# RIKEN-RCCS/GEMMul8

Hardware: AMD Instinct MI355X
Metric: emulated DGEMM TFLOPS (N=8192, moduli=14) (higher is better)
Workload: dtype int8

## Files before the change

### gemmul8_amd/csrc/oz2_driver.hip

```cpp
#include <hip/hip_runtime.h>
#include <stdint.h>
#include <stdio.h>
#include <stdlib.h>
#include <string.h>

#include <algorithm>

#include <atomic>
#include <mutex>

#include "../../include/gemmul8_c.h"
#include "oz2_gemm_common.hpp"
#include "oz2_kernels.h"
#include "oz2_knobs.hpp"

using namespace oz2;

namespace {

inline char* align256(void* p) {
    uintptr_t x = reinterpret_cast<uintptr_t>(p);
    x = (x + 255) & ~uintptr_t(255);
    return reinterpret_cast<char*>(x);
}
inline int norm_op(int op) {
    if (op >= 111 && op <= 113) return op - 111;
    return op;
}
inline size_t low_size(int) { return 1; }
inline size_t mid_size(int backend, bool cplx) { return (backend == kINT8 ? 1 : 2) * (cplx ? 2 : 1); }

static inline bool moduli_ok(int dtype, unsigned N) { return N >= 2 && N <= (is_f32(dtype) ? 13u : 20u); }

static inline bool f8_concat_ok(size_t k, size_t m, size_t n, size_t kp) { return k <= 32768 && 2 * (m + n) * kp <= ((size_t)384 << 20); }

#define OZ2_HIP(expr)                       \
    do {                                    \
        hipError_t e__ = (expr);            \
        if (e__ != hipSuccess) return (int)e__; \
    } while (0)

struct Timer {
    hipEvent_t ev[4];
    bool made = false, ok = false;
};
Timer* thread_timer() {
    constexpr int kMaxDev = 64;
    static thread_local Timer t[kMaxDev];
    int dev = 0;
    if (hipGetDevice(&dev) != hipSuccess || dev < 0 || dev >= kMaxDev) return nullptr;
    Timer& T = t[dev];
    if (!T.made) {
        T.made = T.ok = true;
        for (auto& e : T.ev)
            if (hipEventCreate(&e) != hipSuccess) T.ok = false;
    }
    return T.ok ? &T : nullptr;
}

}

static bool scalars_on_device(const void* alpha);

namespace oz2 {
static Knobs parse_knobs() {
    Knobs k;
    auto num = [](const char* name, int dflt) {
        const char* s = getenv(name);
        return s && *s ? atoi(s) : dflt;
    };
    if (const char* e = getenv("GEMMUL8_EPI_NT"); e && (e[0] == '0' || e[0] == '1') && !e[1]) k.epi_nt = e[0] - '0';
    if (const int t = num("GEMMUL8_BOUND_TILE", 0); t == 128 || t == 256) k.bound_tile = t;
    if (num("GEMMUL8_CPLX_BOUND_LAUNCHES", 1) == 2) k.cplx_bound_launches = 2;
    if (const int c = num("GEMMUL8_CPLX_CHUNK", 0); c >= 1) k.cplx_chunk = c;
    if (const char* e = getenv("GEMMUL8_CRT_KERNEL")) k.crt_kernel = e[0] == 'd' ? 1 : e[0] == 'r' ? 2 : 0;
    if (const int c = num("GEMMUL8_GEMM_CUS", 0); c >= 8) k.gemm_cus = c & ~7;
    if (const char* e = getenv("GEMMUL8_FP8_FUSED"); e && e[0] == '0') k.fp8_fused = 0;
    if (const char* e = getenv("GEMMUL8_FP8_PLANES")) k.fp8_planes = e[0] == 'e' ? 1 : 0;
    if (const char* e = getenv("GEMMUL8_SCALE_FOLD"); e && e[0] == '0') k.scale_fold = 0;
    if (const char* e = getenv("GEMMUL8_BOUNDS_ONE_READ"); e && (e[0] == '0' || e[0] == '1') && !e[1]) k.bounds_one_read = e[0] - '0';
    if (const char* e = getenv("GEMMUL8_CRT_PANELS"); e && atoi(e) > 1) {
        k.crt_panels = std::min(atoi(e), 256);
        k.crt_panels_ring = e[strlen(e) - 1] == 'r';
    }
    if (const char* e = getenv("GEMMUL8_MAP_COLBLOCK"); e && *e) k.map_colblock = atoi(e) > 0 ? atoi(e) : 0;
    return k;
}
static std::atomic<const Knobs*> g_knobs{nullptr};
static std::mutex g_knobs_mtx;
void reload_knobs() {
    std::lock_guard<std::mutex> lk(g_knobs_mtx);
    g_knobs.store(new Knobs(parse_knobs()), std::memory_order_release);
}
const Knobs& knobs() {
    const Knobs* k = g_knobs.load(std::memory_order_acquire);
    if (!k) {
        std::lock_guard<std::mutex> lk(g_knobs_mtx);
        k = g_knobs.load(std::memory_order_acquire);
        if (!k) g_knobs.store(k = new Knobs(parse_knobs()), std::memory_order_release);
    }
    return *k;
}
}

extern "C" {

void gemmul8_reload_knobs(void) { oz2::reload_knobs(); }

static std::atomic<int> g_nonfinite_mode{0};
int gemmul8_set_nonfinite_mode(int mode) {
    if (mode < 0 || mode > 1) return GEMMUL8_E_ARG;
    return g_nonfinite_mode.exchange(mode);
}

int gemmul8_set_fp8_bound_mode(int mode) {
    if (mode < 0 || mode > 2) return GEMMUL8_E_ARG;
    const int old = get_f8_bound_mode();
    set_f8_bound_mode(mode);
    return old;
}

int gemmul8_abi_version(void) { return GEMMUL8_ABI_VERSION; }
size_t gemmul8_layout_bytes(void) { return sizeof(gemmul8_layout); }

const char* gemmul8_version(void) { return "gemmul8-mi355x 0.5 (gfx950; v_mfma_i32_16x16x64_i8 / v_mfma_scale_f32_16x16x128_f8f6f4, fused epilogues)"; }

size_t gemmul8_work_size(int is_complex, int backend, size_t m, size_t n, size_t k, unsigned N, int enA, int enB, size_t* wA,
                         size_t* wB) {
    const size_t kp = padding256(k), mp = padding256(m);
    const size_t sizeA = kp * mp, sizeB = kp * n, sizeC = mp * n;
    const size_t nm = num_mat(backend, N);
    const size_t parts = is_complex ? 3 : 1;
    const size_t midsz = mid_size(backend, is_complex != 0);
    const size_t nhi = (backend == kINT8 ? 1 : 3) * parts;
    const size_t lwork = size_t(1) << 25;
    size_t tA = 255, tB = 255, tC = 255;
    tA += sizeA * (nm + (enA ? 1 : 0)) * parts + 2 * mp;
    tB += sizeB * (nm + (enB ? 1 : 0)) * parts + 2 * padding256(n);
    tC += midsz * sizeC * (N - 1) + std::max(lwork, midsz * sizeC);
    tC += 4 * sizeC * nhi;
    if (wA) *wA = tA;
    if (wB) *wB = tB;
    return tA + tB + tC;
}

int gemmul8_get_layout(int dtype, int backend, size_t m, size_t n, size_t k, unsigned N, void* work, void* workA, void* workB,
                       int enA, int enB, gemmul8_layout* L) {
    if (!L || !work) return GEMMUL8_E_ARG;
    if (!moduli_ok(dtype, N)) return GEMMUL8_E_NUM_MODULI;
    const bool cplx = is_complex(dtype);
    memset(L, 0, sizeof(*L));
    L->kp = padding256(k);
    L->mp = padding256(m);
    L->num_mat = num_mat(backend, N);
    L->parts = cplx ? 3 : 1;
    L->sizeA = L->kp * L->mp;
    L->sizeB = L->kp * n;
    L->sizeC = L->mp * n;
    const size_t offsetA = L->sizeA * L->num_mat, offsetB = L->sizeB * L->num_mat;
    const size_t size_vecA = L->mp, size_vecB = padding256(n);
    char* w = align256(work);
    char* wa = workA ? align256(workA) : nullptr;
    char* wb = workB ? align256(workB) : nullptr;
    char* A_lo = wa ? wa : w;
    char* sftA = A_lo + L->parts * offsetA + (enA ? L->parts * L->sizeA : 0);
    char* B_lo = wb ? wb : (wa ? w : sftA + 2 * size_vecA);
    char* sftB = B_lo + L->parts * offsetB + (enB ? L->parts * L->sizeB : 0);
    char* C_mid = wb ? (wa ? w : sftA + 2 * size_vecA) : sftB + 2 * size_vecB;
    const size_t midsz = mid_size(backend, cplx);
    char* work_native = C_mid + (N - 1) * L->sizeC * midsz;
    const size_t native_sz = std::max(size_t(1) << 25, midsz * L->sizeC);
    char* C_hi = work_native + native_sz;
    const size_t hi_bytes = 4 * L->sizeC * (backend == kINT8 ? 1 : 3) * L->parts;
    L->A_lo = A_lo;
    L->B_lo = B_lo;
    L->part_strideA = offsetA;
    L->part_strideB = offsetB;
    L->A_bound = enA ? A_lo + L->parts * offsetA : A_lo;
    L->B_bound = enB ? B_lo + L->parts * offsetB : B_lo;
    L->sftA = reinterpret_cast<int16_t*>(sftA);
    L->sftB = reinterpret_cast<int16_t*>(sftB);
    L->C_mid = C_mid;
    const size_t tail = (native_sz - midsz * L->sizeC) & ~size_t(255);
    L->scratch = C_hi - tail;
    L->scratch_bytes = tail + hi_bytes;
    L->lo_format = (backend == kFP8 && !enA && !enB && f6_planes_ok(n)) ? 1 : 0;
    return GEMMUL8_OK;
}

static inline size_t scale_fixed_bytes(size_t mp, size_t np) { return (4 * (mp + np) + 2 * (mp + np) + 255) / 256 * 256; }
static inline size_t scale_scratch_bytes(size_t mp, size_t np) { return scale_fixed_bytes(mp, np) + 8 * (mp + np); }
static int scale_scratch(const gemmul8_layout* L, size_t n, int** rowmax, int** colmax, void** amax, int16_t** s0A = nullptr, int16_t** s0B = nullptr) {
    const size_t np = padding256(n);
    if (L->scratch_bytes < scale_scratch_bytes(L->mp, np)) return GEMMUL8_E_ARG;
    *rowmax = (int*)L->scratch;
    *colmax = *rowmax + L->mp;
    int16_t* s0 = (int16_t*)(*colmax + np);
    if (s0A) *s0A = s0;
    if (s0B) *s0B = s0 + L->mp;
    *amax = (char*)L->scratch + scale_fixed_bytes(L->mp, np);
    return GEMMUL8_OK;
}

static int bound_gemm_i8(hipStream_t stream, bool cplx, const gemmul8_layout* L, size_t m, size_t ncols, const int8_t* Ab, const int8_t* Bb, int* rowmax, int* colmax) {
    if (!cplx) {
        const int8_t* As[1] = {Ab};
        const int8_t* Bs[1] = {Bb};
        OZ2_HIP(launch_gemm_i8_max(stream, 1, As, Bs, L->kp, m, ncols, rowmax, colmax));
    } else {
        const int8_t* As[3] = {Ab, Ab + L->sizeA, Ab + 2 * L->sizeA};
        const int8_t* Bs[3] = {Bb + L->sizeB, Bb, Bb + 2 * L->sizeB};
        const bool two_launches = knobs().cplx_bound_launches == 2;
        if (two_launches) {
            OZ2_HIP(launch_gemm_i8_max(stream, 2, As, Bs, L->kp, m, ncols, rowmax, colmax));
            OZ2_HIP(launch_gemm_i8_max(stream, 3, As, Bs, L->kp, m, ncols, rowmax, colmax));
        } else {
            OZ2_HIP(launch_gemm_i8_max(stream, 3, As, Bs, L->kp, m, ncols, rowmax, colmax, 2));
        }
    }
    return GEMMUL8_OK;
}

struct SymSide {
    bool onB;
    int form;
    bool herm;
    bool conj = false;
};
constexpr size_t kOneReadMinRows = 8192;
static int scale_bounds_nf(void* stream_, int dtype, int backend, int op_A, int op_B, size_t m, size_t n, size_t k, const void* A, size_t lda,
                           const void* B, size_t ldb, unsigned N, size_t col_begin, size_t col_end, const gemmul8_layout* L, int skipA, int skipB,
                           bool nf, const SymSide* sym = nullptr) {
    hipStream_t stream = (hipStream_t)stream_;
    if (!L || !A || !B) return GEMMUL8_E_ARG;
    if (!moduli_ok(dtype, N)) return GEMMUL8_E_NUM_MODULI;
    if (backend == kFP8 && k > 65536) return GEMMUL8_E_ARG;
    op_A = norm_op(op_A);
// ... 911 lines not shown
```

### gemmul8_amd/csrc/oz2_gemm_i8.hip

```cpp
#include <hip/hip_runtime.h>
#include <stdint.h>

#include <atomic>
#include <cstdlib>
#include <type_traits>

#include "oz2_crt_common.hpp"
#include "oz2_gemm_common.hpp"
#include "oz2_gemm_i8_epi.hpp"
#include "oz2_kernels.h"

namespace oz2 {

#ifndef OZ2_PB
#define OZ2_PB 4
#endif
#ifndef OZ2_KBAR_MAX_KP
#define OZ2_KBAR_MAX_KP 5120
#endif
#ifndef OZ2_SLEEP_A
#define OZ2_SLEEP_A 4
#endif
#ifndef OZ2_SLEEP_B
#define OZ2_SLEEP_B 4
#endif
constexpr int RING_LDS_BYTES = 5 * TILE_BYTES;

struct NoCrt {
    int unused;
};
#ifdef OZ2_LAB_FUSED_CRT
#include OZ2_LAB_FUSED_CRT
#endif
template <bool ZERO> struct MfmaReinitHook {
    v4i (*acc)[4];
    int acc0;
    __device__ __forceinline__ void operator()(int sb, int phase) const {
        if (phase != 0) return;
        const int tj = sb >> 1, tg = sb & 1;
        const v4i z = {0, 0, 0, 0};
        const v4i c = ZERO ? v4i{0, 0, 0, 0} : v4i{acc0, acc0, acc0, acc0};
        __builtin_amdgcn_sched_barrier(0);
#pragma unroll
        for (int ti = 0; ti < 4; ++ti)
            acc[tg * 4 + ti][tj] = __builtin_amdgcn_mfma_i32_16x16x64_i8(z, acc[tg * 4 + ti][tj], c, 0, 0, 0);
    }
};
#define OZ2_I8_KR 0
#define OZ2_I8_KERNEL_HEAD                                       \
    template <int EPI, bool KBAR, int FUSE, bool SMALLK = false> \
    __global__ void __launch_bounds__(WS_THREADS) gemm_i8_kernel(const GemmArgs args, const std::conditional_t<FUSE != 0, CrtArgs, NoCrt> crt)
#include "oz2_gemm_i8_kernel.inc"
#undef OZ2_I8_KR
#undef OZ2_I8_KERNEL_HEAD
#define OZ2_I8_KR 1
#define OZ2_I8_KERNEL_HEAD                           \
    template <int EPI, bool KBAR, int FUSE, bool SMALLK> \
    __global__ void __launch_bounds__(WS_THREADS) gemm_i8_kr_kernel(const GemmArgs args, const NoCrt crt, const int krange)
#include "oz2_gemm_i8_kernel.inc"
#undef OZ2_I8_KR
#undef OZ2_I8_KERNEL_HEAD

static void fill_common(GemmArgs& a, size_t kp, size_t m, size_t n) {
    a.kp = (int)kp;
    a.m = (int)m;
    a.n = (int)n;
    a.tiles_m = (int)((m + BM - 1) / BM);
    a.tiles_n = (int)((n + BN - 1) / BN);
    for (int t = 0; t < 20; ++t) {
        const int p = GEMMUL8_MODULI_INT8[t];
        a.moduli[t] = p;
        a.pinv32[t] = (int)(4294967296ull / (unsigned long long)p);
        a.dotw[t] = 1u | ((256u % p) << 8) | ((65536u % p) << 16) | ((16777216u % p) << 24);
        a.dotc[t] = (unsigned)((p - (int)(2147483648u % (unsigned)p)) % p);
    }
}

static int num_cus() {
    static int n = 0;
    if (!n) {
        int dev = 0;
        hipDeviceProp_t prop;
        if (hipGetDevice(&dev) != hipSuccess || hipGetDeviceProperties(&prop, dev) != hipSuccess || prop.multiProcessorCount <= 0) return 256;
        n = prop.multiProcessorCount;
    }
    return n;
}

template <int EPI, bool KBAR, int FUSE = 0, bool SMALLK = false, bool KR = false>
static hipError_t launch_sched(hipStream_t stream, GemmArgs& a, const std::conditional_t<FUSE != 0, CrtArgs, NoCrt>& crt = {}, [[maybe_unused]] int krange = 0) {
    static std::atomic<bool> attr_set_dev[64];
    int dev_ = 0;
    if (hipGetDevice(&dev_) != hipSuccess || dev_ < 0 || dev_ >= 64) dev_ = 0;
    if (!attr_set_dev[dev_].load(std::memory_order_acquire)) {
        const void* fn;
        if constexpr (KR) fn = (const void*)gemm_i8_kr_kernel<EPI, KBAR, FUSE, SMALLK>;
        else fn = (const void*)gemm_i8_kernel<EPI, KBAR, FUSE, SMALLK>;
        hipError_t e = hipFuncSetAttribute(fn, hipFuncAttributeMaxDynamicSharedMemorySize, RING_LDS_BYTES);
        if (e != hipSuccess) return e;
        attr_set_dev[dev_].store(true, std::memory_order_release);
    }
    int grid = num_cus() & ~7;
    if (const int want = knobs().gemm_cus; want > 0 && want < grid) grid = want;
    if (grid <= 0) grid = 8;
    if (a.total_tiles < grid) grid = a.total_tiles;
    if constexpr (KR) hipLaunchKernelGGL((gemm_i8_kr_kernel<EPI, KBAR, FUSE, SMALLK>), dim3(grid), dim3(WS_THREADS), RING_LDS_BYTES, stream, a, crt, krange);
    else hipLaunchKernelGGL((gemm_i8_kernel<EPI, KBAR, FUSE, SMALLK>), dim3(grid), dim3(WS_THREADS), RING_LDS_BYTES, stream, a, crt);
    return hipGetLastError();
}

template <int EPI> static hipError_t launch(hipStream_t stream, GemmArgs& a, int planes, int tri = 0, int krange = 0) {
    a.ppi = planes;
    a.m_ppi = map_magic((unsigned)planes);
    a.bstride = g_batch.ws;
    planes *= (int)g_batch.batch;
    if (tri != 0 && (EPI == EPI_MAX || a.tiles_m != a.tiles_n)) return hipErrorInvalidValue;
    if (krange != 0 && (EPI == EPI_MAX || tri != 0 || a.nseg != 1 || g_batch.batch != 1 || krange < kKrALower || krange > kKrBLow)) return hipErrorInvalidValue;
    if (krange != 0 && (krange <= kKrAUpper ? a.tiles_m : a.tiles_n) != a.kp / 256) return hipErrorInvalidValue;
    a.total_tiles = tri ? planes * (a.tiles_m * (a.tiles_m + 1) / 2) : planes * a.tiles_m * a.tiles_n;
    if (a.total_tiles <= 0) return hipSuccess;
    a.colblock = tri ? 0 : map_colblock((size_t)a.tiles_n, (size_t)a.kp * (size_t)a.nseg);
    a.map = tri ? make_tile_map_tri(a.tiles_m, tri) : make_tile_map(a.tiles_m, a.tiles_n, a.colblock);
    a.acc0 = (size_t)a.kp * (size_t)a.nseg <= 512 ? 0 : (int)0x80000000u;
    if constexpr (EPI != EPI_MAX) {
        if (krange != 0) {
            if (a.acc0 == 0) return launch_sched<EPI, true, 0, true, true>(stream, a, {}, krange);
            if (a.kp <= OZ2_KBAR_MAX_KP) return launch_sched<EPI, true, 0, false, true>(stream, a, {}, krange);
            return launch_sched<EPI, false, 0, false, true>(stream, a, {}, krange);
        }
        if (a.acc0 == 0) return launch_sched<EPI, true, 0, true>(stream, a);
        if (a.kp * a.nseg <= OZ2_KBAR_MAX_KP) return launch_sched<EPI, true>(stream, a);
    }
    return launch_sched<EPI, false>(stream, a);
}

static int nt_residue_planes(const GemmArgs& a, int planes, bool stream_out, bool automatic = true) {
    if (const int force = knobs().epi_nt; force >= 0) return force == 1 && stream_out ? planes : 0;
    if (!stream_out || !automatic) return 0;
    const size_t all = (size_t)planes * g_batch.batch;
    const size_t operands = all * (a.strideA + a.strideB), residues = all * a.strideO;
    return residues >= ((size_t)256 << 20) && operands <= ((size_t)240 << 20) ? planes : 0;
}

hipError_t launch_gemm_i8_mod(hipStream_t stream, const int8_t* A, const int8_t* B, size_t strideA, size_t strideB, size_t kp, size_t m,
                              size_t n, int t_begin, int t_end, int8_t* out, size_t ldo, size_t strideO, bool stream_out, int tri, int krange) {
    GemmArgs a{};
    a.A[0] = A;
    a.B[0] = B;
    a.nseg = 1;
    a.strideA = strideA;
    a.strideB = strideB;
    a.t_begin = t_begin;
    a.out = out;
    a.ldo = ldo;
    a.strideO = strideO;
    fill_common(a, kp, m, n);
    a.nt_planes = nt_residue_planes(a, t_end - t_begin, stream_out);
    return launch<EPI_MOD>(stream, a, t_end - t_begin, tri, krange);
}

hipError_t launch_gemm_i8_cplx(hipStream_t stream, const int8_t* A, const int8_t* B, size_t strideA, size_t strideB, size_t kp, size_t m,
                               size_t n, int t_begin, int t_end, const int8_t* rx, const int8_t* ry, size_t strideR, int8_t* out,
                               size_t ldo, size_t strideO, int tri, int krange) {
    GemmArgs a{};
    a.A[0] = A;
    a.B[0] = B;
    a.nseg = 1;
    a.strideA = strideA;
    a.strideB = strideB;
    a.t_begin = t_begin;
    a.out = out;
    a.ldo = ldo;
    a.strideO = strideO;
    a.rx = rx;
    a.ry = ry;
    a.strideR = strideR;
    fill_common(a, kp, m, n);
    a.nt_planes = nt_residue_planes(a, t_end - t_begin, true, false);
    return launch<EPI_CPLX>(stream, a, t_end - t_begin, tri, krange);
}

#ifndef OZ2_MAX_SMALL_TILES
#define OZ2_MAX_SMALL_TILES 128
#endif
hipError_t launch_gemm_i8_max(hipStream_t stream, int nseg, const int8_t* const* A, const int8_t* const* B, size_t kp, size_t m, size_t n,
                              int* rowmax, int* colmax, int mid_seg) {
    {
        const int force = knobs().bound_tile;
        const size_t tiles = ((m + BM - 1) / BM) * ((n + BN - 1) / BN) * g_batch.batch;
        const bool small = force == 128 ? true : force == 256 ? false : tiles <= (size_t)OZ2_MAX_SMALL_TILES;
        if (small) return launch_gemm_i8_max_small(stream, nseg, A, B, kp, m, n, rowmax, colmax, mid_seg);
    }
    GemmArgs a{};
    for (int s = 0; s < nseg; ++s) a.A[s] = A[s], a.B[s] = B[s];
    a.nseg = nseg;
    a.rowmax = rowmax;
    a.colmax = colmax;
    a.kt_mid = mid_seg > 0 && mid_seg < nseg ? mid_seg * (int)(kp / BK) : 0;
    fill_common(a, kp, m, n);
    return launch<EPI_MAX>(stream, a, 1);
}

}
```

### gemmul8_amd/csrc/oz2_gemm_i8_epi.hpp

```cpp
#pragma once
#include <hip/hip_runtime.h>
#include <stdint.h>

#include "oz2_gemm_common.hpp"
#include "oz2_kernels.h"

namespace oz2 {

#if defined(OZ2_PRODUCT_BUILD) && (defined(OZ2_LAB_HOOKS) || defined(OZ2_LAB_FUSED_CRT))
#error "laboratory switches (OZ2_LAB_*) are not allowed in the product build of libgemmul8.so: use tools/experiments/"
#endif
#ifdef OZ2_LAB_HOOKS
#include OZ2_LAB_HOOKS
#endif
#ifndef OZ2_HOOK_DMA_ON
#define OZ2_HOOK_DMA_ON(first_tile) true
#endif
#ifndef OZ2_HOOK_KSTEP
#define OZ2_HOOK_KSTEP(kin) (kin)
#endif
#ifndef OZ2_HOOK_SKIP_EPILOGUE
#define OZ2_HOOK_SKIP_EPILOGUE 0
#endif
#if defined(OZ2_PRODUCT_BUILD) && OZ2_HOOK_SKIP_EPILOGUE
#error "timing probes (OZ2_HOOK_SKIP_*) compute something else: not allowed in the product build of libgemmul8.so"
#endif

enum { EPI_MOD = 0, EPI_MAX = 1, EPI_CPLX = 2 };

struct GemmArgs {
    const int8_t* A[3];
    const int8_t* B[3];
    int nseg;
    size_t strideA;
    size_t strideB;
    int kp;
    int m, n;
    int tiles_m, tiles_n;
    int colblock;
    TileMapArgs map;
    int t_begin;
    int8_t* out;
    size_t ldo;
    size_t strideO;
    const int8_t* rx;
    const int8_t* ry;
    size_t strideR;
    int* rowmax;
    int* colmax;
    int kt_mid;
    int total_tiles;
    int planes;
    int ppi;
    unsigned m_ppi;
    size_t bstride;
    int moduli[20];
    int pinv32[20];
    int nt_planes;
    int acc0;
    unsigned dotw[20];
    unsigned dotc[20];
};

struct PlaneRef {
    size_t boff;
    int tt;
};
template <typename Args> __device__ __forceinline__ PlaneRef plane_ref(const Args& args, int plane) {
    const int p = __builtin_amdgcn_readfirstlane(plane);
    unsigned b, tt;
    udivmod_magic((unsigned)p, (unsigned)args.ppi, args.m_ppi, b, tt);
    return {(size_t)b * args.bstride, (int)tt};
}
struct PlaneConsts {
    int p;
    unsigned dotw, dotc;
};
__device__ __forceinline__ PlaneConsts plane_consts(const GemmArgs& args, PlaneRef pl) {
    const int t = args.t_begin + pl.tt;
    return {args.moduli[t], args.dotw[t], args.dotc[t]};
}
enum { RED_ODD = 1, RED_ODD_SMALL = 3, RED_MAGIC = 4 };
struct NoHook {
    __device__ __forceinline__ void operator()(int, int) const {}
};
typedef unsigned v4u __attribute__((ext_vector_type(4)));
#ifndef OZ2_HOOK_SKIP_STORES
#define OZ2_HOOK_SKIP_STORES 0
#endif
#if defined(OZ2_PRODUCT_BUILD) && OZ2_HOOK_SKIP_STORES
#error "timing probes (OZ2_HOOK_SKIP_*) compute something else: not allowed in the product build of libgemmul8.so"
#endif
template <bool NT> __device__ __forceinline__ void store16_cols(void* ptr, v4u d, int col, int n) {
#if OZ2_HOOK_SKIP_STORES
    asm volatile("" ::"v"(ptr), "v"(d), "v"(col), "s"(n));
    return;
#endif
    unsigned long long saved;
    if constexpr (NT)
        asm volatile("s_mov_b64 %0, exec\n\tv_cmp_gt_i32_e32 vcc, %1, %2\n\ts_and_b64 exec, exec, vcc\n\tglobal_store_dwordx4 %3, %4, off nt\n\ts_nop 1\n\ts_mov_b64 exec, %0"
                     : "=&s"(saved) : "s"(n), "v"(col), "v"(ptr), "v"(d) : "vcc", "scc", "memory");
    else
        asm volatile("s_mov_b64 %0, exec\n\tv_cmp_gt_i32_e32 vcc, %1, %2\n\ts_and_b64 exec, exec, vcc\n\tglobal_store_dwordx4 %3, %4, off\n\ts_nop 1\n\ts_mov_b64 exec, %0"
                     : "=&s"(saved) : "s"(n), "v"(col), "v"(ptr), "v"(d) : "vcc", "scc", "memory");
}
template <int EPI, int RED, typename Hook = NoHook>
__device__ __forceinline__ void i8_epilogue_mod(const v4i (&acc)[8][4], const GemmArgs& args, PlaneRef pl, PlaneConsts pc, int i0, int j0, int lane, Hook hook = {}) {
    const int c16 = lane & 15;
    const int q = lane >> 4;
    const int p = pc.p;
    const float invp = 1.0f / (float)p;
    [[maybe_unused]] const unsigned dotw = pc.dotw, dotc = pc.dotc;
    static_assert(RED == RED_ODD || RED == RED_ODD_SMALL || RED == RED_MAGIC, "one of the three reduction forms");
    [[maybe_unused]] auto red = [&](int x) {
        const float qf = fmaf((float)x, invp, 12582912.0f);
        int r;
        asm("v_mad_i32_i24 %0, %1, %2, %3" : "=v"(r) : "v"(__float_as_int(qf)), "s"(-p), "v"(x));
        return r;
    };
    [[maybe_unused]] const unsigned dotc_f = dotc + 0x4B000000u;
    [[maybe_unused]] auto red_odd_pair = [&](int x0, int x1, int& r0, int& r1) {
        typedef float v2f __attribute__((ext_vector_type(2)));
        const unsigned u0 = __builtin_amdgcn_udot4((unsigned)x0, dotw, dotc_f, false), u1 = __builtin_amdgcn_udot4((unsigned)x1, dotw, dotc_f, false);
        const v2f sm = {__uint_as_float(u0), __uint_as_float(u1)};
        const v2f sf = sm - v2f{8388608.0f, 8388608.0f};
        const v2f qm = __builtin_elementwise_fma(sf, v2f{invp, invp}, v2f{8388608.0f, 8388608.0f});
        asm("v_mad_i32_i24 %0, %1, %2, %3" : "=v"(r0) : "v"(__float_as_int(qm[0])), "s"(-p), "v"(u0));
        asm("v_mad_i32_i24 %0, %1, %2, %3" : "=v"(r1) : "v"(__float_as_int(qm[1])), "s"(-p), "v"(u1));
    };
    [[maybe_unused]] auto red_magic_pair = [&](int x0, int x1, int& r0, int& r1) {
        typedef float v2f __attribute__((ext_vector_type(2)));
        const v2f xm = {__int_as_float(x0), __int_as_float(x1)};
        const v2f xf = xm - v2f{12582912.0f, 12582912.0f};
        const v2f qm = __builtin_elementwise_fma(xf, v2f{invp, invp}, v2f{12582912.0f, 12582912.0f});
        asm("v_mad_i32_i24 %0, %1, %2, %3" : "=v"(r0) : "v"(__float_as_int(qm[0])), "s"(-p), "v"(x0));
        asm("v_mad_i32_i24 %0, %1, %2, %3" : "=v"(r1) : "v"(__float_as_int(qm[1])), "s"(-p), "v"(x1));
    };
    [[maybe_unused]] auto red_small = [&](int x) { return mod_small_sym_odd(x, p, invp); };
    const size_t e00 = (size_t)(j0 + c16) * args.ldo + i0 + q * 16;
    const size_t po = pl.boff + (size_t)pl.tt * args.strideO, pr = pl.boff + (size_t)pl.tt * args.strideR;
    const size_t ejs = (size_t)16 * args.ldo;
    auto reduce_block = [&](int tj, int tg, unsigned (&z)[4]) {
        unsigned d[4];
#pragma unroll
        for (int ti = 0; ti < 4; ++ti) {
            int r[4];
            if constexpr (RED == RED_ODD) {
                red_odd_pair(acc[tg * 4 + ti][tj][0], acc[tg * 4 + ti][tj][1], r[0], r[1]);
                red_odd_pair(acc[tg * 4 + ti][tj][2], acc[tg * 4 + ti][tj][3], r[2], r[3]);
            } else if constexpr (RED == RED_MAGIC) {
                red_magic_pair(acc[tg * 4 + ti][tj][0], acc[tg * 4 + ti][tj][1], r[0], r[1]);
                red_magic_pair(acc[tg * 4 + ti][tj][2], acc[tg * 4 + ti][tj][3], r[2], r[3]);
            } else {
#pragma unroll
                for (int b = 0; b < 4; ++b) r[b] = red(acc[tg * 4 + ti][tj][b]);
            }
            d[ti] = __builtin_amdgcn_perm((unsigned)r[1], (unsigned)r[0], 0x0c0c0400u) |
                    __builtin_amdgcn_perm((unsigned)r[3], (unsigned)r[2], 0x04000c0cu);
        }
        const auto s0 = __builtin_amdgcn_permlane32_swap(d[0], d[2], false, false);
        const auto s1 = __builtin_amdgcn_permlane32_swap(d[1], d[3], false, false);
        const auto w01 = __builtin_amdgcn_permlane16_swap(s0[0], s1[0], false, false);
        const auto w23 = __builtin_amdgcn_permlane16_swap(s0[1], s1[1], false, false);
        z[0] = w01[0], z[1] = w01[1], z[2] = w23[0], z[3] = w23[1];
    };
    if constexpr (EPI == EPI_MOD) {
#pragma unroll
        for (int tj = 0; tj < 4; ++tj) {
            const int col = j0 + tj * 16 + c16;
#pragma unroll
            for (int tg = 0; tg < 2; ++tg) {
                unsigned z[4];
                reduce_block(tj, tg, z);
                hook(2 * tj + tg, 0);
                const size_t e = e00 + tj * ejs + tg * 64;
                if (pl.tt < args.nt_planes) store16_cols<true>(args.out + po + e, v4u{z[0], z[1], z[2], z[3]}, col, args.n);
                else store16_cols<false>(args.out + po + e, v4u{z[0], z[1], z[2], z[3]}, col, args.n);
// ... 119 lines not shown
```

### gemmul8_amd/csrc/oz2_gemm_i8_kernel.inc

```
OZ2_I8_KERNEL_HEAD {
#ifndef OZ2_LAB_FUSED_CRT
    static_assert(FUSE == 0, "the in-kernel CRT forms are laboratory code: tools/experiments/fused_crt");
#endif
    static_assert(FUSE == 0 || EPI == EPI_MOD, "the CRT tail follows the real requantise epilogue");
    static_assert(offsetof(CrtArgs, Cmid) == 0 && alignof(CrtArgs) == 8, "i8_crt_tail locates the block in the kernel-argument segment");
    (void)crt;
#if OZ2_I8_KR
    static_assert(EPI != EPI_MAX && FUSE == 0, "K ranges: residue launches of a single K segment");
#define OZ2_I8_MAP_TILE(vb_) map_tile<true, true>((vb_), total, args.map)
#define OZ2_I8_KSTEPS(tmap_) tile_ksteps(tmap_)
#else
#define OZ2_I8_MAP_TILE(vb_) map_tile<EPI != EPI_MAX>((vb_), total, args.map)
#define OZ2_I8_KSTEPS(tmap_) KT
#endif
    const int planes_per_tile = FUSE ? args.planes : 1;
    extern __shared__ __attribute__((aligned(16))) char smem[];
    const int tid = threadIdx.x;
    const int lane = tid & 63;
    const int wave = __builtin_amdgcn_readfirstlane(tid >> 6);
    const int KT1 = args.kp / BK;
    const int KT = KT1 * args.nseg;
    const int total = args.total_tiles;
    const int G = gridDim.x;
#if OZ2_I8_KR
// ... 58 lines not shown
        for (int vb = blockIdx.x; vb < total; vb += G) {
#if OZ2_I8_KR
            const int nk = OZ2_I8_KSTEPS(OZ2_I8_MAP_TILE(vb));
            for (int kt = 0; kt < nk; ++kt) {
#else
            for (int kt = 0; kt < KT * planes_per_tile; ++kt) {
#endif
                const bool issued = more && OZ2_HOOK_DMA_ON(vb == (int)blockIdx.x);
                if (issued) PRODUCER_BEGIN();
#pragma unroll
                for (int sl = 0; sl < 8; ++sl) {
                    if (issued) {
                        if (isB) {
                            constexpr int PB = OZ2_PB;
#pragma unroll
                            for (int q = 0; q < 16; ++q)
                                if (q * PB / 16 == sl) PRODUCER_DMA(fsrc, q, fdst);
                        } else {
#pragma unroll
                            for (int q = 0; q < 2; ++q) PRODUCER_DMA(fsrc, sl * 2 + q, fdst);
                        }
                    }
                    if (sl == 7 && issued) PRODUCER_ADVANCE();
                    if (sl == 7) {
                        if (!isB && issued) asm volatile("s_waitcnt vmcnt(16)" ::: "memory");
                        else asm volatile("s_waitcnt vmcnt(0)" ::: "memory");
                    }
                    __builtin_amdgcn_s_barrier();
                }
            }
        }
        __builtin_amdgcn_s_barrier();
        }
#include "oz2_gemm_i8_producer_undef.inc"
        return;
    }

    const int wm = wave >> 2, wn = wave & 3;
    const int r16 = lane & 15;
    const int q = lane >> 4;
    const int sw = (r16 >> 1) & 7;
    const int a_base = (wm * 128 + r16) * BK;
    const int b_base = (wn * 64 + r16) * BK;

    if constexpr (KBAR) {
    __builtin_amdgcn_s_barrier();
    auto run = [&]<bool WM1>() {
        int sA = 0;
        constexpr bool MFMA_REINIT = SMALLK && EPI == EPI_MOD && FUSE == 0;
        v4i acc[8][4];
        if constexpr (MFMA_REINIT) {
#pragma unroll
            for (int i = 0; i < 8; ++i)
#pragma unroll
                for (int j = 0; j < 4; ++j) acc[i][j] = v4i{args.acc0, args.acc0, args.acc0, args.acc0};
        }
        for (int vb = blockIdx.x; vb < total; vb += G) {
            const TileMap tmap = OZ2_I8_MAP_TILE(vb);
            const PlaneRef pref = (FUSE || EPI == EPI_MAX) ? PlaneRef{0, 0} : plane_ref(args, tmap.plane);
            const PlaneConsts pcon = (FUSE || EPI == EPI_MAX) ? PlaneConsts{} : plane_consts(args, pref);
            for (int pl = 0; pl < planes_per_tile; ++pl) {
            v4i af[4], bf[4];
            if constexpr (!MFMA_REINIT) {
#pragma unroll
            for (int i = 0; i < 8; ++i)
#pragma unroll
                for (int j = 0; j < 4; ++j)
                    acc[i][j] = v4i{EPI == EPI_MAX ? 0 : args.acc0, EPI == EPI_MAX ? 0 : args.acc0, EPI == EPI_MAX ? 0 : args.acc0, EPI == EPI_MAX ? 0 : args.acc0};
            }
#define OZ2_KBAR_PIN() __builtin_amdgcn_sched_barrier(0)
#define OZ2_KBAR_WAIT() do {} while (0)
#define OZ2_LOAD_SEG(seg_)                                                                                                   \
    do {                                                                                                                     \
        const int coff_ = (((((seg_) >> 1) << 2) | q) ^ sw) << 4;                                                            \
        if (((seg_) & 1) == 0) {                                                                                             \
            _Pragma("unroll") for (int j = 0; j < 4; ++j) bf[j] = *(const v4i*)(curB + j * 16 * BK + coff_);                 \
        }                                                                                                                    \
        _Pragma("unroll") for (int i = 0; i < 4; ++i) { af[i] = *(const v4i*)(curA + (((seg_) & 1) * 4 + i) * 16 * BK + coff_); OZ2_KBAR_PIN(); } \
    } while (0)
#define OZ2_MMA_SEG(seg_)                                                                                            \
    do {                                                                                                                     \
        OZ2_KBAR_WAIT();                                                                   \
        __builtin_amdgcn_sched_barrier(0);                                                                                   \
        __builtin_amdgcn_s_setprio(1);                                                                                       \
        _Pragma("unroll") for (int i = 0; i < 4; ++i) _Pragma("unroll") for (int jj = 0; jj < 4; ++jj) {                     \
            const int j = (i & 1) ? 3 - jj : jj;                                    \
            acc[((seg_) & 1) * 4 + i][j] = __builtin_amdgcn_mfma_i32_16x16x64_i8(af[i], bf[j], acc[((seg_) & 1) * 4 + i][j], 0, 0, 0); \
        }                                                                                                                    \
        __builtin_amdgcn_s_setprio(0);                                                                                       \
        __builtin_amdgcn_sched_barrier(0);                                                                                   \
    } while (0)
#define OZ2_SET_PANELS()                                                                                                     \
    const char* curA = smem + sA * TILE_BYTES + a_base;                                                                      \
    const char* curB = smem + (sA == 4 ? 0 : sA + 1) * TILE_BYTES + b_base;                                                  \
    sA = sA + 2 >= 5 ? sA - 3 : sA + 2
            int kt = 0;
            const int nph = (EPI == EPI_MAX && args.kt_mid > 0) ? 2 : 1;
            for (int ph = 0; ph < nph; ++ph) {
            const int kt_end = (EPI == EPI_MAX && ph + 1 < nph) ? args.kt_mid : OZ2_I8_KSTEPS(tmap);
            auto kstep = [&]() {
                OZ2_SET_PANELS();
#pragma unroll
                for (int seg = 0; seg < 4; ++seg) {
                    OZ2_LOAD_SEG(seg);
                    if (WM1 && seg == 3) {
                        asm volatile("s_waitcnt lgkmcnt(0)" ::: "memory");
                        __builtin_amdgcn_sched_barrier(0);
                        __builtin_amdgcn_s_barrier();
                        __builtin_amdgcn_sched_barrier(0);
                    }
                    OZ2_MMA_SEG(seg);
                }
                if (!WM1) {
                    __builtin_amdgcn_s_barrier();
                    __builtin_amdgcn_sched_barrier(0);
                }
            };
            for (; kt < kt_end; ++kt) kstep();
#undef OZ2_SET_PANELS
#undef OZ2_LOAD_SEG
#undef OZ2_MMA_SEG
#undef OZ2_KBAR_PIN
#undef OZ2_KBAR_WAIT
#if OZ2_HOOK_SKIP_EPILOGUE
            (void)tmap;
#pragma unroll
            for (int i = 0; i < 8; ++i)
#pragma unroll
                for (int j = 0; j < 4; ++j) asm volatile("" ::"v"(acc[i][j]));
#else
            int lane_e = lane;
            if constexpr (EPI == EPI_MOD) {
            asm volatile("v_mbcnt_lo_u32_b32 %0, -1, 0\n\tv_mbcnt_hi_u32_b32 %0, -1, %0" : "=v"(lane_e));
            } else {
                __builtin_amdgcn_s_waitcnt(0x0F70);
            }
            if constexpr (FUSE != 0) i8_epilogue<EPI, NoHook, -1>(acc, args, PlaneRef{0, pl}, tmap.tm * BM + (WM1 ? 128 : 0), tmap.tn * BN + wn * 64, lane_e);
            else if constexpr (EPI == EPI_MAX) i8_epilogue<EPI, NoHook, 0>(acc, args, plane_ref(args, tmap.plane), PlaneConsts{}, tmap.tm * BM + (WM1 ? 128 : 0), tmap.tn * BN + wn * 64, lane_e);
            else if constexpr (MFMA_REINIT) i8_epilogue<EPI, MfmaReinitHook<true>, (int)SMALLK>(acc, args, pref, pcon, tmap.tm * BM + (WM1 ? 128 : 0), tmap.tn * BN + wn * 64, lane_e, MfmaReinitHook<true>{acc, args.acc0});
            else i8_epilogue<EPI, NoHook, (int)SMALLK>(acc, args, pref, pcon, tmap.tm * BM + (WM1 ? 128 : 0), tmap.tn * BN + wn * 64, lane_e);
#endif
            }
            }
            if constexpr (FUSE != 0) asm volatile("s_waitcnt vmcnt(0)" ::: "memory");
        }
        if constexpr (FUSE != 0) __builtin_amdgcn_s_barrier();
    };
    if (wm == 0) run.template operator()<false>();
    else run.template operator()<true>();
    } else {
    __builtin_amdgcn_s_barrier();
    if (wm == 1) __builtin_amdgcn_s_barrier();
    int sA = 0;
    for (int vb = blockIdx.x; vb < total; vb += G) {
        const TileMap tmap = OZ2_I8_MAP_TILE(vb);
        const PlaneRef pref = (FUSE || EPI == EPI_MAX) ? PlaneRef{0, 0} : plane_ref(args, tmap.plane);
        const PlaneConsts pcon = (FUSE || EPI == EPI_MAX) ? PlaneConsts{} : plane_consts(args, pref);
        for (int pl = 0; pl < planes_per_tile; ++pl) {
        v4i acc[8][4];
#pragma unroll
        for (int i = 0; i < 8; ++i)
#pragma unroll
            for (int j = 0; j < 4; ++j)
                acc[i][j] = v4i{EPI == EPI_MAX ? 0 : args.acc0, EPI == EPI_MAX ? 0 : args.acc0, EPI == EPI_MAX ? 0 : args.acc0, EPI == EPI_MAX ? 0 : args.acc0};

        int kt = 0;
        const int nph = (EPI == EPI_MAX && args.kt_mid > 0) ? 2 : 1;
        for (int ph = 0; ph < nph; ++ph) {
        const int kt_end = (EPI == EPI_MAX && ph + 1 < nph) ? args.kt_mid : OZ2_I8_KSTEPS(tmap);
        for (; kt < kt_end; ++kt) {
            const char* curA = smem + sA * TILE_BYTES + a_base;
            const char* curB = smem + (sA == 4 ? 0 : sA + 1) * TILE_BYTES + b_base;
            sA = sA + 2 >= 5 ? sA - 3 : sA + 2;
#pragma unroll
            for (int ks2 = 0; ks2 < 2; ++ks2) {
                const int coff = (((ks2 << 2) | q) ^ sw) << 4;
                v4i bf[4];
#pragma unroll
                for (int ah = 0; ah < 2; ++ah) {
                    v4i af[4];
                    if (ah == 0) {
#pragma unroll
                        for (int j = 0; j < 4; ++j)
                            bf[j] = *(const v4i*)(curB + j * 16 * BK + coff);
                    }
#pragma unroll
                    for (int i = 0; i < 4; ++i)
                        af[i] = *(const v4i*)(curA + (ah * 4 + i) * 16 * BK + coff);
                    if (ks2 == 1 && ah == 1) asm volatile("s_waitcnt lgkmcnt(0)" ::: "memory");
                    __builtin_amdgcn_sched_barrier(0);
                    __builtin_amdgcn_s_barrier();
                    __builtin_amdgcn_sched_barrier(0);
                    if (!(ks2 == 1 && ah == 1)) asm volatile("s_waitcnt lgkmcnt(0)" ::: "memory");
                    __builtin_amdgcn_sched_barrier(0);
                    __builtin_amdgcn_s_setprio(1);
#pragma unroll
                    for (int i = 0; i < 4; ++i)
#pragma unroll
                        for (int jj = 0; jj < 4; ++jj) {
                            const int j = (i & 1) ? 3 - jj : jj;
                            acc[ah * 4 + i][j] = __builtin_amdgcn_mfma_i32_16x16x64_i8(af[i], bf[j], acc[ah * 4 + i][j], 0, 0, 0);
                        }
                    __builtin_amdgcn_s_setprio(0);
                    __builtin_amdgcn_sched_barrier(0);
                    __builtin_amdgcn_s_barrier();
                    __builtin_amdgcn_sched_barrier(0);
                }
            }
        }
#if OZ2_HOOK_SKIP_EPILOGUE
        (void)tmap;
#pragma unroll
        for (int i = 0; i < 8; ++i)
#pragma unroll
            for (int j = 0; j < 4; ++j) asm volatile("" ::"v"(acc[i][j]));
#else
        __builtin_amdgcn_s_waitcnt(0x0F70);
        if constexpr (FUSE != 0) i8_epilogue<EPI, NoHook, -1>(acc, args, PlaneRef{0, pl}, tmap.tm * BM + wm * 128, tmap.tn * BN + wn * 64, lane);
        else if constexpr (EPI == EPI_MAX) i8_epilogue<EPI, NoHook, 0>(acc, args, plane_ref(args, tmap.plane), PlaneConsts{}, tmap.tm * BM + wm * 128, tmap.tn * BN + wn * 64, lane);
        else i8_epilogue<EPI, NoHook, (int)SMALLK>(acc, args, pref, pcon, tmap.tm * BM + wm * 128, tmap.tn * BN + wn * 64, lane);
#endif
        }
        }
#ifdef OZ2_LAB_FUSED_CRT
        if constexpr (FUSE != 0) i8_crt_tail<std::conditional_t<FUSE == 2, float, double>>(args, tmap.tm * BM + wm * 128, tmap.tn * BN + wn * 64, lane);
#endif
    }
    if (wm == 0) __builtin_amdgcn_s_barrier();
    }
}
#undef OZ2_I8_MAP_TILE
#undef OZ2_I8_KSTEPS
```

### gemmul8_amd/csrc/oz2_knobs.hpp

```cpp
#pragma once

namespace oz2 {

struct Knobs {
    int epi_nt = -1;
    int bound_tile = 0;
    int cplx_bound_launches = 1;
    int cplx_chunk = 0;
    int crt_kernel = 0;
    int fp8_planes = 0;
    int fp8_fused = 1;
    int gemm_cus = 0;
    int crt_panels = 0;
    int crt_panels_ring = 0;
    int scale_fold = 1;
    int bounds_one_read = -1;
    int map_colblock = -1;
};
const Knobs& knobs();
void reload_knobs();

}
```

Baseline: 161.3.

## Add side-by-side epilogue variant of ping-pong int8 GEMM for residue launches

Adds a gemm_i8_sbs_kernel variant in which the two wave groups run offset by one k-step: wm==1 defers its final barrier and re-syncs at the next tile. This lets the epilogues of the two halves overlap with the other half's MFMA work instead of both stalling at once. It is enabled by default for EPI_MOD launches with at most 1024 output tiles, and can be forced on or off with the GEMMUL8_GEMM_SBS environment variable. The barrier count is rebalanced with an extra s_barrier at kernel end, which risks deadlock or mismatched barriers if a grid or tile edge case is wrong. It also adds a half-epilogue-skip timing probe macro, guarded against product builds.

Measured after the change: 163.1 (median of 6 runs). +1.1%, better.

```diff
diff --git a/gemmul8_amd/csrc/oz2_driver.hip b/gemmul8_amd/csrc/oz2_driver.hip
--- a/gemmul8_amd/csrc/oz2_driver.hip
+++ b/gemmul8_amd/csrc/oz2_driver.hip
@@ -83,6 +83,7 @@
         k.crt_panels = std::min(atoi(e), 256);
         k.crt_panels_ring = e[strlen(e) - 1] == 'r';
     }
+    if (const char* e = getenv("GEMMUL8_GEMM_SBS"); e && (e[0] == '0' || e[0] == '1')) k.gemm_sbs = e[0] - '0';
     if (const char* e = getenv("GEMMUL8_MAP_COLBLOCK"); e && *e) k.map_colblock = atoi(e) > 0 ? atoi(e) : 0;
     return k;
 }
diff --git a/gemmul8_amd/csrc/oz2_gemm_i8.hip b/gemmul8_amd/csrc/oz2_gemm_i8.hip
--- a/gemmul8_amd/csrc/oz2_gemm_i8.hip
+++ b/gemmul8_amd/csrc/oz2_gemm_i8.hip
@@ -17,6 +17,12 @@
 #endif
 #ifndef OZ2_KBAR_MAX_KP
 #define OZ2_KBAR_MAX_KP 5120
+#endif
+#ifndef OZ2_SBS_DEFAULT
+#define OZ2_SBS_DEFAULT 1
+#endif
+#ifndef OZ2_SBS_MAX_TILES
+#define OZ2_SBS_MAX_TILES 1024
 #endif
 #ifndef OZ2_SLEEP_A
 #define OZ2_SLEEP_A 4
@@ -47,10 +53,20 @@
     }
 };
 #define OZ2_I8_KR 0
+#define OZ2_I8_SBS 0
 #define OZ2_I8_KERNEL_HEAD                                       \
     template <int EPI, bool KBAR, int FUSE, bool SMALLK = false> \
     __global__ void __launch_bounds__(WS_THREADS) gemm_i8_kernel(const GemmArgs args, const std::conditional_t<FUSE != 0, CrtArgs, NoCrt> crt)
 #include "oz2_gemm_i8_kernel.inc"
+#undef OZ2_I8_KERNEL_HEAD
+#undef OZ2_I8_SBS
+#define OZ2_I8_SBS 1
+#define OZ2_I8_KERNEL_HEAD                               \
+    template <int EPI, bool KBAR, int FUSE, bool SMALLK> \
+    __global__ void __launch_bounds__(WS_THREADS) gemm_i8_sbs_kernel(const GemmArgs args, const NoCrt crt)
+#include "oz2_gemm_i8_kernel.inc"
+#undef OZ2_I8_SBS
+#define OZ2_I8_SBS 0
 #undef OZ2_I8_KR
 #undef OZ2_I8_KERNEL_HEAD
 #define OZ2_I8_KR 1
@@ -59,6 +75,7 @@
     __global__ void __launch_bounds__(WS_THREADS) gemm_i8_kr_kernel(const GemmArgs args, const NoCrt crt, const int krange)
 #include "oz2_gemm_i8_kernel.inc"
 #undef OZ2_I8_KR
+#undef OZ2_I8_SBS
 #undef OZ2_I8_KERNEL_HEAD
 
 static void fill_common(GemmArgs& a, size_t kp, size_t m, size_t n) {
@@ -87,7 +104,7 @@
     return n;
 }
 
-template <int EPI, bool KBAR, int FUSE = 0, bool SMALLK = false, bool KR = false>
+template <int EPI, bool KBAR, int FUSE = 0, bool SMALLK = false, bool KR = false, bool SBS = false>
 static hipError_t launch_sched(hipStream_t stream, GemmArgs& a, const std::conditional_t<FUSE != 0, CrtArgs, NoCrt>& crt = {}, [[maybe_unused]] int krange = 0) {
     static std::atomic<bool> attr_set_dev[64];
     int dev_ = 0;
@@ -95,6 +112,7 @@
     if (!attr_set_dev[dev_].load(std::memory_order_acquire)) {
         const void* fn;
         if constexpr (KR) fn = (const void*)gemm_i8_kr_kernel<EPI, KBAR, FUSE, SMALLK>;
+        else if constexpr (SBS) fn = (const void*)gemm_i8_sbs_kernel<EPI, KBAR, FUSE, SMALLK>;
         else fn = (const void*)gemm_i8_kernel<EPI, KBAR, FUSE, SMALLK>;
         hipError_t e = hipFuncSetAttribute(fn, hipFuncAttributeMaxDynamicSharedMemorySize, RING_LDS_BYTES);
         if (e != hipSuccess) return e;
@@ -105,6 +123,7 @@
     if (grid <= 0) grid = 8;
     if (a.total_tiles < grid) grid = a.total_tiles;
     if constexpr (KR) hipLaunchKernelGGL((gemm_i8_kr_kernel<EPI, KBAR, FUSE, SMALLK>), dim3(grid), dim3(WS_THREADS), RING_LDS_BYTES, stream, a, crt, krange);
+    else if constexpr (SBS) hipLaunchKernelGGL((gemm_i8_sbs_kernel<EPI, KBAR, FUSE, SMALLK>), dim3(grid), dim3(WS_THREADS), RING_LDS_BYTES, stream, a, crt);
     else hipLaunchKernelGGL((gemm_i8_kernel<EPI, KBAR, FUSE, SMALLK>), dim3(grid), dim3(WS_THREADS), RING_LDS_BYTES, stream, a, crt);
     return hipGetLastError();
 }
@@ -131,6 +150,9 @@
         if (a.acc0 == 0) return launch_sched<EPI, true, 0, true>(stream, a);
         if (a.kp * a.nseg <= OZ2_KBAR_MAX_KP) return launch_sched<EPI, true>(stream, a);
     }
+    if constexpr (EPI == EPI_MOD) {
+        if (const int sbs = knobs().gemm_sbs; sbs == 1 || (sbs < 0 && OZ2_SBS_DEFAULT && a.tiles_m * a.tiles_n <= OZ2_SBS_MAX_TILES)) return launch_sched<EPI_MOD, false, 0, false, false, true>(stream, a);
+    }
     return launch_sched<EPI, false>(stream, a);
 }
 
diff --git a/gemmul8_amd/csrc/oz2_gemm_i8_epi.hpp b/gemmul8_amd/csrc/oz2_gemm_i8_epi.hpp
--- a/gemmul8_amd/csrc/oz2_gemm_i8_epi.hpp
+++ b/gemmul8_amd/csrc/oz2_gemm_i8_epi.hpp
@@ -22,7 +22,10 @@
 #ifndef OZ2_HOOK_SKIP_EPILOGUE
 #define OZ2_HOOK_SKIP_EPILOGUE 0
 #endif
-#if defined(OZ2_PRODUCT_BUILD) && OZ2_HOOK_SKIP_EPILOGUE
+#ifndef OZ2_HOOK_SKIP_EPILOGUE_HALF
+#define OZ2_HOOK_SKIP_EPILOGUE_HALF 0
+#endif
+#if defined(OZ2_PRODUCT_BUILD) && (OZ2_HOOK_SKIP_EPILOGUE || OZ2_HOOK_SKIP_EPILOGUE_HALF)
 #error "timing probes (OZ2_HOOK_SKIP_*) compute something else: not allowed in the product build of libgemmul8.so"
 #endif
 
diff --git a/gemmul8_amd/csrc/oz2_gemm_i8_kernel.inc b/gemmul8_amd/csrc/oz2_gemm_i8_kernel.inc
--- a/gemmul8_amd/csrc/oz2_gemm_i8_kernel.inc
+++ b/gemmul8_amd/csrc/oz2_gemm_i8_kernel.inc
@@ -234,6 +234,9 @@
     __builtin_amdgcn_s_barrier();
     if (wm == 1) __builtin_amdgcn_s_barrier();
     int sA = 0;
+#if OZ2_I8_SBS
+    static_assert(EPI == EPI_MOD && !KBAR && FUSE == 0 && !SMALLK && !OZ2_I8_KR, "side-by-side epilogues: the residue launch of the ping-pong schedule, one phase per tile");
+#endif
     for (int vb = blockIdx.x; vb < total; vb += G) {
         const TileMap tmap = OZ2_I8_MAP_TILE(vb);
         const PlaneRef pref = (FUSE || EPI == EPI_MAX) ? PlaneRef{0, 0} : plane_ref(args, tmap.plane);
@@ -245,51 +248,38 @@
 #pragma unroll
             for (int j = 0; j < 4; ++j)
                 acc[i][j] = v4i{EPI == EPI_MAX ? 0 : args.acc0, EPI == EPI_MAX ? 0 : args.acc0, EPI == EPI_MAX ? 0 : args.acc0, EPI == EPI_MAX ? 0 : args.acc0};
+#if OZ2_I8_SBS
+        if (wm == 1 && vb != (int)blockIdx.x) {
+#pragma unroll
+            for (int i = 0; i < 8; ++i)
+#pragma unroll
+                for (int j = 0; j < 4; ++j) asm volatile("" : "+v"(acc[i][j]));
+            __builtin_amdgcn_sched_barrier(0);
+            __builtin_amdgcn_s_barrier();
+            __builtin_amdgcn_sched_barrier(0);
+        }
+#endif
 
         int kt = 0;
         const int nph = (EPI == EPI_MAX && args.kt_mid > 0) ? 2 : 1;
         for (int ph = 0; ph < nph; ++ph) {
         const int kt_end = (EPI == EPI_MAX && ph + 1 < nph) ? args.kt_mid : OZ2_I8_KSTEPS(tmap);
+#define OZ2_I8_PP_DEFER 0
+#if OZ2_I8_SBS
+        for (; kt < kt_end - wm; ++kt) {
+#else
         for (; kt < kt_end; ++kt) {
-            const char* curA = smem + sA * TILE_BYTES + a_base;
-            const char* curB = smem + (sA == 4 ? 0 : sA + 1) * TILE_BYTES + b_base;
-            sA = sA + 2 >= 5 ? sA - 3 : sA + 2;
-#pragma unroll
-            for (int ks2 = 0; ks2 < 2; ++ks2) {
-                const int coff = (((ks2 << 2) | q) ^ sw) << 4;
-                v4i bf[4];
-#pragma unroll
-                for (int ah = 0; ah < 2; ++ah) {
-                    v4i af[4];
-                    if (ah == 0) {
-#pragma unroll
-                        for (int j = 0; j < 4; ++j)
-                            bf[j] = *(const v4i*)(curB + j * 16 * BK + coff);
-                    }
-#pragma unroll
-                    for (int i = 0; i < 4; ++i)
-                        af[i] = *(const v4i*)(curA + (ah * 4 + i) * 16 * BK + coff);
-                    if (ks2 == 1 && ah == 1) asm volatile("s_waitcnt lgkmcnt(0)" ::: "memory");
-                    __builtin_amdgcn_sched_barrier(0);
-                    __builtin_amdgcn_s_barrier();
-                    __builtin_amdgcn_sched_barrier(0);
-                    if (!(ks2 == 1 && ah == 1)) asm volatile("s_waitcnt lgkmcnt(0)" ::: "memory");
-                    __builtin_amdgcn_sched_barrier(0);
-                    __builtin_amdgcn_s_setprio(1);
-#pragma unroll
-                    for (int i = 0; i < 4; ++i)
-#pragma unroll
-                        for (int jj = 0; jj < 4; ++jj) {
-                            const int j = (i & 1) ? 3 - jj : jj;
-                            acc[ah * 4 + i][j] = __builtin_amdgcn_mfma_i32_16x16x64_i8(af[i], bf[j], acc[ah * 4 + i][j], 0, 0, 0);
-                        }
-                    __builtin_amdgcn_s_setprio(0);
-                    __builtin_amdgcn_sched_barrier(0);
-                    __builtin_amdgcn_s_barrier();
-                    __builtin_amdgcn_sched_barrier(0);
-                }
-            }
-        }
+#endif
+#include "oz2_gemm_i8_pp_kstep.inc"
+        }
+#undef OZ2_I8_PP_DEFER
+#if OZ2_I8_SBS
+        if (wm == 1) {
+#define OZ2_I8_PP_DEFER 1
+#include "oz2_gemm_i8_pp_kstep.inc"
+#undef OZ2_I8_PP_DEFER
+        }
+#endif
 #if OZ2_HOOK_SKIP_EPILOGUE
         (void)tmap;
 #pragma unroll
@@ -297,17 +287,36 @@
 #pragma unroll
             for (int j = 0; j < 4; ++j) asm volatile("" ::"v"(acc[i][j]));
 #else
+#if OZ2_HOOK_SKIP_EPILOGUE_HALF
+        if ((OZ2_HOOK_SKIP_EPILOGUE_HALF >> wm) & 1) {
+#pragma unroll
+            for (int i = 0; i < 8; ++i)
+#pragma unroll
+                for (int j = 0; j < 4; ++j) asm volatile("" ::"v"(acc[i][j]));
+        } else
+#endif
+        {
         __builtin_amdgcn_s_waitcnt(0x0F70);
+#if OZ2_I8_SBS
+        int lane_e;
+        asm volatile("v_mbcnt_lo_u32_b32 %0, -1, 0\n\tv_mbcnt_hi_u32_b32 %0, -1, %0" : "=v"(lane_e));
+        i8_epilogue<EPI, NoHook, (int)SMALLK>(acc, args, pref, pcon, tmap.tm * BM + wm * 128, tmap.tn * BN + wn * 64, lane_e);
+#else
         if constexpr (FUSE != 0) i8_epilogue<EPI, NoHook, -1>(acc, args, PlaneRef{0, pl}, tmap.tm * BM + wm * 128, tmap.tn * BN + wn * 64, lane);
         else if constexpr (EPI == EPI_MAX) i8_epilogue<EPI, NoHook, 0>(acc, args, plane_ref(args, tmap.plane), PlaneConsts{}, tmap.tm * BM + wm * 128, tmap.tn * BN + wn * 64, lane);
         else i8_epilogue<EPI, NoHook, (int)SMALLK>(acc, args, pref, pcon, tmap.tm * BM + wm * 128, tmap.tn * BN + wn * 64, lane);
 #endif
         }
+#endif
+        }
         }
 #ifdef OZ2_LAB_FUSED_CRT
         if constexpr (FUSE != 0) i8_crt_tail<std::conditional_t<FUSE == 2, float, double>>(args, tmap.tm * BM + wm * 128, tmap.tn * BN + wn * 64, lane);
 #endif
     }
+#if OZ2_I8_SBS
+    if (wm == 1 && (int)blockIdx.x < total) __builtin_amdgcn_s_barrier();
+#endif
     if (wm == 0) __builtin_amdgcn_s_barrier();
     }
 }
diff --git a/gemmul8_amd/csrc/oz2_gemm_i8_pp_kstep.inc b/gemmul8_amd/csrc/oz2_gemm_i8_pp_kstep.inc
--- /dev/null
+++ b/gemmul8_amd/csrc/oz2_gemm_i8_pp_kstep.inc
@@ -0,0 +1,41 @@
+            const char* curA = smem + sA * TILE_BYTES + a_base;
+            const char* curB = smem + (sA == 4 ? 0 : sA + 1) * TILE_BYTES + b_base;
+            sA = sA + 2 >= 5 ? sA - 3 : sA + 2;
+#pragma unroll
+            for (int ks2 = 0; ks2 < 2; ++ks2) {
+                const int coff = (((ks2 << 2) | q) ^ sw) << 4;
+                v4i bf[4];
+#pragma unroll
+                for (int ah = 0; ah < 2; ++ah) {
+                    v4i af[4];
+                    if (ah == 0) {
+#pragma unroll
+                        for (int j = 0; j < 4; ++j)
+                            bf[j] = *(const v4i*)(curB + j * 16 * BK + coff);
+                    }
+#pragma unroll
+                    for (int i = 0; i < 4; ++i)
+                        af[i] = *(const v4i*)(curA + (ah * 4 + i) * 16 * BK + coff);
+                    if (ks2 == 1 && ah == 1) asm volatile("s_waitcnt lgkmcnt(0)" ::: "memory");
+                    __builtin_amdgcn_sched_barrier(0);
+                    __builtin_amdgcn_s_barrier();
+                    __builtin_amdgcn_sched_barrier(0);
+                    if (!(ks2 == 1 && ah == 1)) asm volatile("s_waitcnt lgkmcnt(0)" ::: "memory");
+                    __builtin_amdgcn_sched_barrier(0);
+                    __builtin_amdgcn_s_setprio(1);
+#pragma unroll
+                    for (int i = 0; i < 4; ++i)
+#pragma unroll
+                        for (int jj = 0; jj < 4; ++jj) {
+                            const int j = (i & 1) ? 3 - jj : jj;
+                            acc[ah * 4 + i][j] = __builtin_amdgcn_mfma_i32_16x16x64_i8(af[i], bf[j], acc[ah * 4 + i][j], 0, 0, 0);
+                        }
+                    __builtin_amdgcn_s_setprio(0);
+                    __builtin_amdgcn_sched_barrier(0);
+#if OZ2_I8_PP_DEFER
+                    if (!(ks2 == 1 && ah == 1))
+#endif
+                    __builtin_amdgcn_s_barrier();
+                    __builtin_amdgcn_sched_barrier(0);
+                }
+            }
diff --git a/gemmul8_amd/csrc/oz2_knobs.hpp b/gemmul8_amd/csrc/oz2_knobs.hpp
--- a/gemmul8_amd/csrc/oz2_knobs.hpp
+++ b/gemmul8_amd/csrc/oz2_knobs.hpp
@@ -15,6 +15,7 @@
     int crt_panels_ring = 0;
     int scale_fold = 1;
     int bounds_one_read = -1;
+    int gemm_sbs = -1;
     int map_colblock = -1;
 };
 const Knobs& knobs();
```
